# tgm-team/tgm

Hardware: AMD Instinct MI355X
Metric: sampled-edges/sec (TGAT 2-hop k=20 recency sampler, tgbl-wiki synthetic) (higher is better)
Workload: dtype int32/int64 indices + f32 feature rows (copied, no arithmetic)

## Files before the change

include/tgm_amd.h:

```cpp
#ifndef TGM_AMD_H
#define TGM_AMD_H

#include <stddef.h>
#include <stdint.h>

#ifdef __cplusplus
extern "C" {
#endif

#define TGMX_ABI_VERSION 7

#define TGMX_OK 0
#define TGMX_E_INVALID (-1)
#define TGMX_E_LAUNCH (-2)
#define TGMX_E_UNSUPPORTED (-3)

#define TGMX_ST_SEED_RANGE 1
#define TGMX_ST_SEED_TIME 2
#define TGMX_ST_EDGE_RANGE 4
#define TGMX_ST_SCRATCH 8
#define TGMX_ST_TS_BOUND 16

typedef void* tgmx_stream_t;
typedef void* tgmx_event_t;
// ... 80 lines not shown
  int64_t ts_bound;
  int32_t neg_group, neg_low, neg_high;
  uint64_t neg_seed, neg_call;
  int32_t* neg_out;
  int64_t* neg_time_out;
  int32_t guard_seed_errors;
  int32_t sorted_ts;
  int32_t* out_valid[TGMX_MAX_HOPS];
  int32_t* out_valid_prev[TGMX_MAX_HOPS];
  int64_t neg_index0;
  int64_t* csr_cursor;
  int32_t csr_x_by_pos;
  int32_t* out_eid[TGMX_MAX_HOPS];
  struct tgmx_defer* defer;
  int32_t defer_ok;
} tgmx_recency_step_t;

int tgmx_recency_step(const tgmx_recency_step_t* step, tgmx_stream_t stream);
#define TGMX_PLAN_FUSED01 1
#define TGMX_RIDE_NONE 0
#define TGMX_RIDE_SORT 1
#define TGMX_RIDE_MERGE 2
#define TGMX_RIDE_SORT_MERGE 3
#define TGMX_RIDE_PLACE_ONLY 4
#define TGMX_RIDE_ALL 5
#define TGMX_RIDE_SORT_MERGE_PLACE 6
#define TGMX_RIDE_MERGE_PLACE 7
#define TGMX_AFTER_NONE 0
#define TGMX_AFTER_COMMIT 1
#define TGMX_AFTER_PRESORTED 2
#define TGMX_AFTER_MERGE_PRESORTED 3
#define TGMX_AFTER_BLOCK 4
#define TGMX_AFTER_LARGE 5
int tgmx_recency_step_plan(const tgmx_recency_step_t* step);
// ... 28 lines not shown
} tgmx_pipeline_t;

typedef struct tgmx_pipeline_out {
  int32_t* neg;
  int64_t* neg_time;
  int32_t* seed_nid0;
  int64_t* seed_ts0;
  int32_t* out_nid[TGMX_MAX_HOPS];
  int64_t* out_ts[TGMX_MAX_HOPS];
  float* out_x[TGMX_MAX_HOPS];
  int32_t timed_hop;
  tgmx_event_t ev_start, ev_stop;
  int32_t* out_valid[TGMX_MAX_HOPS];
  int32_t* out_valid_prev[TGMX_MAX_HOPS];
  int32_t* out_eid[TGMX_MAX_HOPS];
} tgmx_pipeline_out_t;

typedef struct tgmx_pipeline_post {
  int32_t dedup;
  int32_t dedup_neg, dedup_nbr;
  int32_t num_nodes;
  void* dedup_ws;
  int32_t* uniq_out;
  int32_t edge_hop;
  int64_t edge_cap;
  int64_t* row_off;
  int64_t* edge_index;
  int64_t* edge_t;
  float* edge_x;
  int64_t* dev_sizes;
// ... 1032 lines not shown
```

tgm_amd/_native.py:

```python
from __future__ import annotations

import ctypes
import os
from ctypes import c_char_p, c_int32, c_int64, c_size_t, c_void_p
from typing import Optional

import torch

from .exceptions import NativeLibraryError

_HERE = os.path.dirname(os.path.abspath(__file__))
LIB_PATH = os.path.join(_HERE, 'csrc', 'libtgm_amd.so')

_P = c_void_p
SIGNATURES = {
    'tgmx_version': (c_int32, []),
    'tgmx_abi_sizeof': (c_size_t, [c_int32]),
    'tgmx_last_error': (c_char_p, []),
    'tgmx_event_create': (c_int32, [ctypes.POINTER(c_void_p)]),
    'tgmx_event_destroy': (c_int32, [_P]),
    'tgmx_event_elapsed_ms': (c_int32, [_P, _P, ctypes.POINTER(ctypes.c_float)]),
    'tgmx_recency_lookup_csr': (
        c_int32,
        [_P, _P, _P, c_int32, _P, _P, c_int64, c_int32, c_int32, c_int64, c_int64, c_int32, c_int32, _P, _P, _P, _P, _P, _P, _P],
# ... 129 lines not shown
        ('n_groups', c_int32),
        ('grp_nid', c_void_p * MAX_SEED_GROUPS), ('grp_ts', c_void_p * MAX_SEED_GROUPS), ('grp_n', c_int64 * MAX_SEED_GROUPS),
        ('seed_nid0', c_void_p), ('seed_ts0', c_void_p), ('S0', c_int64),
        ('n_hops', c_int32), ('k', c_int32 * MAX_HOPS),
        ('out_nid', c_void_p * MAX_HOPS), ('out_ts', c_void_p * MAX_HOPS), ('out_x', c_void_p * MAX_HOPS),
        ('src', c_void_p), ('dst', c_void_p), ('ts', c_void_p), ('edge_x', c_void_p),
        ('n', c_int64), ('eid0', c_int64), ('directed', c_int32), ('key_wrap32', c_int32),
        ('scratch', c_void_p), ('status', c_void_p),
        ('timed_hop', c_int32), ('ev_start', c_void_p), ('ev_stop', c_void_p),
        ('ts_bound', c_int64),
        ('neg_group', c_int32), ('neg_low', c_int32), ('neg_high', c_int32),
        ('neg_seed', ctypes.c_uint64), ('neg_call', ctypes.c_uint64), ('neg_out', c_void_p), ('neg_time_out', c_void_p),
        ('guard_seed_errors', c_int32), ('sorted_ts', c_int32),
        ('out_valid', c_void_p * MAX_HOPS), ('out_valid_prev', c_void_p * MAX_HOPS),
        ('neg_index0', c_int64), ('csr_cursor', c_void_p), ('csr_x_by_pos', c_int32), ('out_eid', c_void_p * MAX_HOPS),
        ('defer', c_void_p), ('defer_ok', c_int32),
    ]


class PipelinePost(ctypes.Structure):

    _fields_ = [
        ('dedup', c_int32), ('dedup_neg', c_int32), ('dedup_nbr', c_int32), ('num_nodes', c_int32), ('dedup_ws', c_void_p), ('uniq_out', c_void_p),
        ('edge_hop', c_int32), ('edge_cap', c_int64), ('row_off', c_void_p), ('edge_index', c_void_p), ('edge_t', c_void_p), ('edge_x', c_void_p),
        ('dev_sizes', c_void_p), ('host_sizes', c_void_p), ('sizes_ready', c_void_p),
    ]


class TgnMemoryFwd(ctypes.Structure):

    _fields_ = [
# ... 164 lines not shown
    _fields_ = [
        ('src', c_void_p), ('dst', c_void_p), ('ts', c_void_p), ('edge_x', c_void_p), ('num_edges', c_int64),
        ('rank', c_int32), ('world', c_int32), ('n_roles', c_int32), ('seed_role', c_int32 * MAX_SEED_GROUPS),
        ('neg_low', c_int32), ('neg_high', c_int32), ('neg_seed', ctypes.c_uint64),
        ('update', c_int32), ('reserved0', c_int32), ('step', RecencyStep),
    ]


class PipelineOut(ctypes.Structure):

    _fields_ = [
        ('neg', c_void_p), ('neg_time', c_void_p), ('seed_nid0', c_void_p), ('seed_ts0', c_void_p),
        ('out_nid', c_void_p * MAX_HOPS), ('out_ts', c_void_p * MAX_HOPS), ('out_x', c_void_p * MAX_HOPS),
        ('timed_hop', c_int32), ('ev_start', c_void_p), ('ev_stop', c_void_p),
        ('out_valid', c_void_p * MAX_HOPS), ('out_valid_prev', c_void_p * MAX_HOPS), ('out_eid', c_void_p * MAX_HOPS),
    ]


ACCOUNTING_PARTIALS = 1024
SIGNATURES['tgmx_lookup_accounting'] = (c_int32, [_P, c_int64, _P, _P, c_int64, _P, _P])
SIGNATURES['tgmx_uniform_lookup_csr'] = (c_int32, [_P, _P, _P, c_int32, _P, c_int64, c_int32, c_int64, c_int32, c_int32, ctypes.c_uint64, ctypes.c_uint64,
                                                   _P, _P, _P, _P, _P])
SIGNATURES['tgmx_ring_update_scratch_bytes'] = (c_size_t, [c_int64, c_int32])
SIGNATURES['tgmx_defer_create'] = (c_void_p, [c_int32, c_int32])
SIGNATURES['tgmx_defer_destroy'] = (None, [_P])
SIGNATURES['tgmx_defer_pending'] = (c_int32, [_P])
SIGNATURES['tgmx_defer_count'] = (c_int64, [_P])
SIGNATURES['tgmx_defer_flush'] = (c_int32, [_P, _P])
SIGNATURES['tgmx_set_fused_rows'] = (c_int32, [c_int32])
SIGNATURES['tgmx_set_fused_order'] = (c_int32, [c_int32])
SIGNATURES['tgmx_fused_row_order'] = (c_int32, [c_int64, c_int32, c_int32, _P, c_int32, _P])
SIGNATURES['tgmx_tgn_gru_gate_backward'] = (c_int32, [_P, _P, _P, _P, c_int32, c_int64, _P, _P, _P])
SIGNATURES['tgmx_tgn_aggregate_backward'] = (c_int32, [c_int64, _P, _P, _P, _P, _P, _P, c_int32, c_int32, _P, _P, c_int32, c_int32, _P, _P, _P])
SIGNATURES['tgmx_tconv_edge_attr_backward'] = (c_int32, [_P, _P, _P, _P, _P, _P, c_int32, c_int32, c_int64, _P, _P])
# ... 633 lines not shown
```

tgm_amd/csrc/pipeline.hip:

```cpp
#include <algorithm>

#include "common.h"

using namespace tgmx;

__global__ __launch_bounds__(64) void sizes_to_host_kernel(const int64_t* __restrict__ dev, int64_t* __restrict__ host) {
  if (threadIdx.x < 3) __hip_atomic_store(&host[threadIdx.x], dev[threadIdx.x], __ATOMIC_RELAXED, __HIP_MEMORY_SCOPE_SYSTEM);
}

static int pipeline_post(const tgmx_pipeline_t* p, const tgmx_recency_step_t& s, int64_t edge_lo, int64_t n_edges, long long share,
                         const tgmx_pipeline_out_t* out, const tgmx_pipeline_post_t* post, tgmx_stream_t stream) {
  TGMX_REQUIRE(post->dev_sizes && post->host_sizes && post->sizes_ready, "pipeline_step: post block needs dev_sizes / host_sizes / sizes_ready");
  long long rows[TGMX_MAX_HOPS + 1];
  rows[0] = share * p->n_roles;
  for (int h = 0; h < s.n_hops; ++h) rows[h + 1] = rows[h] * s.k[h];
  bool scan_rides = false;
  if (post->dedup) {
    TGMX_REQUIRE(post->dedup_ws && post->uniq_out, "pipeline_step: null dedup buffer");
    const int32_t* parts[16];
    int64_t sizes[16];
    int np = 0;
    parts[np] = p->src + edge_lo; sizes[np++] = n_edges;
    parts[np] = p->dst + edge_lo; sizes[np++] = n_edges;
    if (post->dedup_neg && s.neg_out) { parts[np] = s.neg_out; sizes[np++] = share; }
// ... 63 lines not shown
        s.neg_index0 = lo;
        s.neg_out = out->neg; s.neg_time_out = out->neg_time;
        break;
      default: TGMX_REQUIRE(false, "pipeline_step: seed role %d", p->seed_role[g]);
    }
  }
  s.seed_nid0 = out->seed_nid0;
  s.seed_ts0 = out->seed_ts0;
  for (int h = 0; h < s.n_hops && h < TGMX_MAX_HOPS; ++h) {
    s.out_nid[h] = out->out_nid[h];
    s.out_ts[h] = out->out_ts[h];
    s.out_x[h] = out->out_x[h];
    s.out_valid[h] = out->out_valid[h];
    s.out_valid_prev[h] = out->out_valid_prev[h];
    s.out_eid[h] = out->out_eid[h];
  }
  s.timed_hop = out->timed_hop;
  s.ev_start = out->ev_start;
  s.ev_stop = out->ev_stop;
  if (s.indptr) {
    s.ev_hi = edge_lo;
    s.n = 0;
  } else if (p->update && n_edges > 0) {
    s.src = p->src + edge_lo;
    s.dst = p->dst + edge_lo;
    s.ts = p->ts + edge_lo;
    s.edge_x = (p->edge_x && s.D > 0) ? p->edge_x + edge_lo * (long long)s.D : nullptr;
    s.n = n_edges;
    s.eid0 = edge_lo;
    s.defer_ok = 1;
// ... 58 lines not shown
```

tgm_amd/csrc/recency.hip:

```cpp
#include <algorithm>
#include <atomic>
#include <cstdlib>
#include <cstring>
#include <string>
#include <vector>

#include <hip/hip_ext.h>
#include <rocprim/block/block_radix_sort.hpp>
#include <rocprim/block/block_scan.hpp>
#include <rocprim/device/device_radix_sort.hpp>
#include <rocprim/device/device_scan.hpp>
#include <rocprim/iterator/counting_iterator.hpp>
#include <rocprim/iterator/transform_iterator.hpp>

#include "common.h"

namespace tgmx {

struct __align__(16) Rec {
  int nbr;
  int eid;
  long long ts;
};
static_assert(sizeof(Rec) == sizeof(tgmx_adj_t), "record layout");
// ... 108 lines not shown
  unsigned commit_blocks;
  const unsigned long long* phdr;
  const Rec* prec;
  const int32_t* pslot;
  const float* pstore;
  unsigned pstamp;
  int peid0;
  int k1;
  int32_t* out_nid1;
  int64_t* out_ts1;
  float* out_x1;
  int32_t* out_valid;
  int32_t* out_valid1;
  int32_t* out_valid_prev;
  int32_t* out_valid_prev1;
  int fused_rows;
  FusedOrder ord;
  long long* ts;
};

template <int VEC>
struct VecOf;
template <>
struct VecOf<4> { using type = float4; };
template <>
struct VecOf<2> { using type = float2; };
template <>
struct VecOf<1> { using type = float; };

template <typename T>
// ... 1123 lines not shown
      has[u] = e >= 0;
      const bool st = e >= lim;
      ptr[u] = (st ? P : X) + (has[u] ? (long long)(st ? e - lim : e) * a.row_vecs + col : 0);
    }
    V v[U];
#pragma unroll
    for (int u = 0; u < U; ++u) v[u] = *ptr[u];
#pragma unroll
    for (int u = 0; u < U; ++u) {
      const int f = f0 + u * kWave;
      if (f < total) O[f] = has[u] ? v[u] : zero_vec<V>();
    }
  }
}

template <bool RING, int VEC, bool SMALL, bool PRE = false>
__device__ __forceinline__ void lookup_seed(const LookupArgs& a, long long s, int n, long long q, int k, int lane, int* lds_eid,
                                            int32_t* out_nid, int64_t* out_ts, float* out_x, int32_t* out_valid, int32_t* out_valid_prev,
                                            int32_t* out_eid = nullptr, int v_old_pre = 0) {
  const bool live = n >= 0 && n < a.N;
  int v_new = 0;
  if (SMALL) {
    const SmallPick o = small_pick<RING>(a, n, q, k, live, lane);
    if (lane < k) {
      out_nid[s * k + lane] = o.nbr;
      out_ts[s * k + lane] = o.ts;
      if (out_eid) out_eid[s * k + lane] = o.eid;
      lds_eid[lane] = o.src;
    }
    const unsigned long long m = __ballot(lane < k && o.has);
    v_new = m ? k - __builtin_ctzll(m) : 0;
  } else {
    const int B = a.B;
    const Window w = find_window<RING>(a, n, live, lane);
    int cnt = 0;
    for (int top = w.wlen; top > 0 && cnt == 0; top -= kWave) {
      const int lo = top > kWave ? top - kWave : 0;
      const int i = lo + lane;
      bool ok = false;
      if (i < top) {
        const Rec r = a.recs[slot_of<RING>(w, B, i)];
        ok = r.nbr >= 0 && r.ts < q;
      }
      const unsigned long long m = __ballot(ok);
      if (m) cnt = lo + 64 - __clzll((long long)m);
    }
    for (int c = lane; c < k; c += kWave) {
      const int i = cnt - k + c;
      Rec r;
      r.nbr = -1; r.eid = 0; r.ts = 0;
      if (i >= 0) r = a.recs[slot_of<RING>(w, B, i)];
      const bool has = r.nbr >= 0;
      out_nid[s * k + c] = has ? r.nbr : -1;
      out_ts[s * k + c] = has ? r.ts : 0;
      if (out_eid) out_eid[s * k + c] = has ? r.eid : -1;
      lds_eid[c] = has ? ((RING || a.x_by_pos) ? (int)slot_of<RING>(w, B, i) : r.eid) : -1;
      if (has && k - c > v_new) v_new = k - c;
    }
    for (int o = 32; o > 0; o >>= 1) {
      const int other = __shfl_xor(v_new, o);
      v_new = other > v_new ? other : v_new;
    }
  }
  if (a.D == 0 || out_x == nullptr) return;
  int first_slot = 0;
  if (out_valid) {
    const int v_old = PRE ? v_old_pre : out_valid[s];
    first_slot = k - (v_old > v_new ? v_old : v_new);
    if (lane == 0) {
      out_valid[s] = v_new;
      if (out_valid_prev) out_valid_prev[s] = v_old;
    }
  }
  __builtin_amdgcn_wave_barrier();
  gather_rows<VEC>(a, s, k, lane, lds_eid, out_x, first_slot);
  __builtin_amdgcn_wave_barrier();
}

template <bool RING, int VEC, bool SMALL, bool RIDE>
__global__ __launch_bounds__(256) void recency_lookup_kernel(const LookupArgs a, const UpdateArgs u) {
  extern __shared__ __attribute__((aligned(16))) int lds_eid_all[];
  unsigned bid = blockIdx.x, nblk = gridDim.x;
  if constexpr (RING && RIDE) {
    if (bid < a.side_blocks) {
      update_side_work(u, a.side_stage, (int)bid);
      return;
    }
    bid -= a.side_blocks;
    nblk -= a.side_blocks;
  }
  const int lane = lane_id();
  const int wave_in_block = threadIdx.x >> 6;
  int* lds_eid = lds_eid_all + wave_in_block * a.k;
  const long long waves_total = (long long)nblk * (blockDim.x >> 6);
  for (long long s = (long long)bid * (blockDim.x >> 6) + wave_in_block; s < a.S; s += waves_total) {
    int n;
    long long q;
    fetch_seed(a, s, lane, true, n, q);
    check_seed(a, n, q, a.allow_pad, lane);
    lookup_seed<RING, VEC, SMALL>(a, s, n, q, a.k, lane, lds_eid, a.out_nid, a.out_ts, a.out_x, a.out_valid, a.out_valid_prev, a.out_eid);
  }
}

constexpr int kFusedTsWords = 8;
constexpr int kFusedRowsDefault = 0;
enum FusedTsRole : long long { kTsRider = 1, kTsCommit = 2, kTsHop0 = 3, kTsHop1 = 4 };
__device__ __forceinline__ long long ts_after(int v) {
  asm volatile("" ::"v"(v));
  return (long long)wall_clock64();
}

template <bool RING>
__device__ __forceinline__ SmallPick fused_row_pick(const LookupArgs& a, const PickLoads& L, int n, long long q, bool live, int lane) {
  if constexpr (RING) return pick_finish(a, L, n, q, a.k1, live, lane);
  else return small_pick<false>(a, n, q, a.k1, live, lane);
// ... 33 lines not shown
  const int k0 = a.k, k1 = a.k1;
  int* lds_eid = lds_eid_all + wave_in_block * (k0 > k1 ? k0 : k1);
  const long long waves_total = (long long)nblk * (blockDim.x >> 6);
  const long long S0 = a.S;
  const int G = ROWS ? a.fused_rows : 0;
  const int runs = G > 0 ? (k0 + G - 1) / G : k0;
  long long role = 0, t_seed = 0, t_index = 0, t_gather = 0, ts_row = -1;
  for (long long w = (long long)bid * (blockDim.x >> 6) + wave_in_block; w < S0 + S0 * runs; w += waves_total) {
    int n;
    long long q;
    if (w < S0) {
      role = kTsHop0;
      if constexpr (ROWS) {
        fetch_seed(a, w, lane, true, n, q);
        check_seed(a, n, q, 0, lane);
        lookup_seed<RING, VEC, true>(a, w, n, q, k0, lane, lds_eid, a.out_nid, a.out_ts, a.out_x, a.out_valid, a.out_valid_prev, a.out_eid);
      } else {
        const int v_old = (a.D > 0 && a.out_x && a.out_valid) ? a.out_valid[w] : 0;
        fetch_seed(a, w, lane, true, n, q);
        check_seed(a, n, q, 0, lane);
        lookup_seed<RING, VEC, true, true>(a, w, n, q, k0, lane, lds_eid, a.out_nid, a.out_ts, a.out_x, a.out_valid, a.out_valid_prev, a.out_eid, v_old);
      }
    } else if (!ROWS) {
      role = kTsHop1;
      long long s0;
      int j;
      fused_row_of(a.ord, w - S0, k0, S0, s0, j);
      const long long idx = s0 * k0 + j;
      const int v_old = (a.D > 0 && a.out_x1 && a.out_valid1) ? a.out_valid1[idx] : 0;
      if (TS) ts_row = idx;
      int n0;
      long long q0;
      fetch_seed(a, s0, lane, false, n0, q0);
      const SmallPick o = small_pick<RING>(a, n0, q0, k0, n0 >= 0 && n0 < a.N, lane);
      n = __shfl(o.nbr, j);
      q = __shfl(o.ts, j);
      lookup_seed<RING, VEC, true, true>(a, idx, n, q, k1, lane, lds_eid, a.out_nid1, a.out_ts1, a.out_x1, a.out_valid1, a.out_valid_prev1, a.out_eid1, v_old);
    } else {
      const long long run = w - S0;
      const long long s0 = run / runs;
      const int j0 = (int)(run - s0 * runs) * G;
      const int rows = k0 - j0 < G ? k0 - j0 : G;
      const long long base = s0 * k0 + j0;
      const bool feats = a.D > 0 && a.out_x1 != nullptr;
      const int v_old_run = (feats && a.out_valid1 && lane < rows) ? a.out_valid1[base + lane] : 0;
      int n0;
      long long q0;
      fetch_seed(a, s0, lane, false, n0, q0);
      const SmallPick o0 = small_pick<RING>(a, n0, q0, k0, n0 >= 0 && n0 < a.N, lane);
      n = __shfl(o0.nbr, j0);
      q = __shfl(o0.ts, j0);
      bool live = n >= 0 && n < a.N;
// ... 2 lines not shown
        t_seed = ts_after(n);
      }
      PickLoads L = RING ? pick_issue(a, n, live, lane) : PickLoads{};
      for (int r = 0; r < rows; ++r) {
        const long long s = base + r;
        const long long t0 = TS ? (long long)wall_clock64() : 0;
        const SmallPick o = fused_row_pick<RING>(a, L, n, q, live, lane);
        if (lane < k1) {
          a.out_nid1[s * k1 + lane] = o.nbr;
          a.out_ts1[s * k1 + lane] = o.ts;
          if (a.out_eid1) a.out_eid1[s * k1 + lane] = o.eid;
          lds_eid[lane] = o.src;
        }
        const unsigned long long m = __ballot(lane < k1 && o.has);
        const int v_new = m ? k1 - __builtin_ctzll(m) : 0;
        if (TS) {
          const long long t1 = ts_after(v_new);
          t_index += t1 - t0;
        }
        if (r + 1 < rows) {
          n = __shfl(o0.nbr, j0 + r + 1);
          q = __shfl(o0.ts, j0 + r + 1);
          live = n >= 0 && n < a.N;
          if (RING) L = pick_issue(a, n, live, lane);
        }
        if (!feats) continue;
        int first_slot = 0;
        if (a.out_valid1) {
          const int v_old = __shfl(v_old_run, r);
          first_slot = k1 - (v_old > v_new ? v_old : v_new);
          if (lane == 0) {
            a.out_valid1[s] = v_new;
            if (a.out_valid_prev1) a.out_valid_prev1[s] = v_old;
          }
        }
        const long long t2 = TS ? (long long)wall_clock64() : 0;
        __builtin_amdgcn_wave_barrier();
        gather_rows<VEC>(a, s, k1, lane, lds_eid, a.out_x1, first_slot);
        __builtin_amdgcn_wave_barrier();
        if (TS) t_gather += (long long)wall_clock64() - t2;
      }
    }
  }
  if (TS && lane == 0) {
    ts_rec[0] = t_start;
    ts_rec[1] = (long long)wall_clock64();
    ts_rec[2] = role;
    ts_rec[3] = t_seed;
// ... 673 lines not shown
  a.row_vecs = a.D > 0 ? a.D / vec : 1;
  a.dv = make_fastdiv((uint32_t)a.row_vecs);
  a.dv_seed = make_fastdiv((uint32_t)(kmax * a.row_vecs));
  if ((unsigned long long)kmax * a.row_vecs * (unsigned long long)a.row_vecs >= (1ull << 32)) {
    set_error("recency_lookup: k*D^2 too large for the slot divider (k=%d, D=%d)", kmax, a.D);
    return TGMX_E_UNSUPPORTED;
  }
  return vec;
}

static int packed_group_lanes(const LookupArgs& a, int k, bool ring) {
  const int gl = (a.B <= 16 && k <= 16) ? 16 : ((a.B <= 32 && k <= 32) ? 32 : 64);
  return (ring && gl < 64 && (long long)k * a.row_vecs <= 8 * gl) ? gl : 64;
}

template <bool RING>
static int launch_lookup(LookupArgs a, hipStream_t stream, hipEvent_t ev_start, hipEvent_t ev_stop,
                         const UpdateArgs* side = nullptr, int side_stage = 0, unsigned side_blocks = 0) {
  if (a.S == 0) return TGMX_OK;
  const UpdateArgs u = side ? *side : UpdateArgs{};
  a.side_blocks = (RING && side) ? side_blocks : 0;
  a.side_stage = side_stage;
  const bool small = a.B <= kWave && a.k <= kWave;
  const int vec = prepare_lookup(a, a.out_x, a.k);
  if (vec < 0) return vec;
  const int waves_per_block = 4;
  long long blocks = (a.S + waves_per_block - 1) / waves_per_block;
  if (blocks > (1 << 20)) blocks = 1 << 20;
  const dim3 grid((unsigned)blocks + a.side_blocks), block(waves_per_block * kWave);
  const size_t lds = (size_t)waves_per_block * a.k * sizeof(int);
  const bool ride = RING && a.side_blocks > 0;
#define TGMX_LAUNCH(VEC_, SMALL_)                                                                                              \
  do {                                                                                                                         \
    if (ride) TGMX_LAUNCH_TIMED((recency_lookup_kernel<RING, VEC_, SMALL_, true>), grid, block, lds, stream, ev_start, ev_stop, a, u); \
    else TGMX_LAUNCH_TIMED((recency_lookup_kernel<RING, VEC_, SMALL_, false>), grid, block, lds, stream, ev_start, ev_stop, a, u);     \
  } while (0)
  const int gl_any = a.out_eid ? 64 : packed_group_lanes(a, a.k, true);
  static const bool packed_hop0 = !(getenv("TGMX_PACKED_HOP0") && atoi(getenv("TGMX_PACKED_HOP0")) == 0);
  const int gl = (a.grp.groups == 0 || packed_hop0) ? gl_any : 64;
  static const bool tile_on = !(getenv("TGMX_TILE") && atoi(getenv("TGMX_TILE")) == 0);
  const bool tile_ok = gl_any < 64 && tile_on && a.B <= 32 && a.k <= 32 && (((uintptr_t)a.out_nid | (uintptr_t)a.out_ts) & 15) == 0 &&
                       a.S <= (1ll << 25) && a.S >= 2ll * kWave * device_cu_count() &&
                       (!RING || (long long)a.N * a.B * (a.D > 0 ? a.D : 1) * 4 < (1ll << 32) - 64);
  if (tile_ok) {
    const int wpb = ride ? 4 : 1;
    const long long tiles = (a.S + kWave - 1) / kWave;
    long long tblocks = (tiles + wpb - 1) / wpb;
    if (a.leave_room && !ride) {
      const long long room = (long long)device_cu_count() * 12;
      if (tblocks > room) tblocks = room;
    }
    const dim3 tgrid((unsigned)tblocks + a.side_blocks), tblock(wpb * kWave);
// ... 989 lines not shown
  if (n_hops == 1) return {{kSideSort}, {chunks}, 0, kAfterMergePresorted};
  if (chunks == 1) return {{kSideSortMerge, kSidePlaceOnly}, {1, 1}, 0, kAfterCommit};
  if (m <= kRidePlaceMaxM) return {{kSideSort, kSideMergePlace}, {chunks, chunks}, 0, kAfterCommit};
  return {{kSideSort, kSideMerge}, {chunks, chunks}, 0, kAfterPresorted};
}

static long long hop0_seed_count(const tgmx_recency_step_t* s) {
  if (s->n_groups <= 0) return s->S0;
  long long S = 0;
  for (int g = 0; g < s->n_groups && g < TGMX_MAX_SEED_GROUPS; ++g) S += s->grp_n[g];
  return S;
}

static long long ring_entries(const tgmx_recency_step_t* s) { return s->n <= 0 ? 0 : (s->directed ? s->n : 2 * s->n); }

extern "C" int tgmx_recency_step_plan(const tgmx_recency_step_t* s) {
  if (!s) return 0;
  const long long S = hop0_seed_count(s);
  const bool fused = plan_fuse01(s, S);
  const RiderPlan p = plan_riders(ring_entries(s), s->n_hops, S, fused, s->indptr == nullptr);
  return (fused ? TGMX_PLAN_FUSED01 : 0) | p.stage[0] << 4 | p.stage[1] << 8 | (int)p.blocks[0] << 12 | (int)p.blocks[1] << 17 |
         (p.pcap / 512) << 22 | p.after << 24;
}

static LookupArgs step_lookup_args(const tgmx_recency_step_t* s) {
  LookupArgs a{};
  a.indptr = s->indptr; a.recs = reinterpret_cast<const Rec*>(s->ring); a.write_pos = s->write_pos; a.edge_x = s->ring_x;
  a.status = s->status; a.D = s->D; a.B = s->B; a.N = s->num_nodes;
  a.ev_lo = s->ev_lo; a.ev_hi = s->ev_hi;
  a.x_by_pos = s->indptr && s->csr_x_by_pos;
  return a;
}

extern "C" int tgmx_recency_step(const tgmx_recency_step_t* s, tgmx_stream_t stream) {
  TGMX_REQUIRE(s, "recency_step: null argument block");
  TGMX_REQUIRE(s->n_groups >= 0 && s->n_groups <= TGMX_MAX_SEED_GROUPS && s->n_hops >= 0 && s->n_hops <= TGMX_MAX_HOPS,
// ... 78 lines not shown

  const int32_t* cur_n = s->seed_nid0;
  const int64_t* cur_t = s->seed_ts0;
  int h = 0;
  if (fused) {
    const int k0 = s->k[0], k1 = s->k[1];
    TGMX_REQUIRE(s->B >= k0 && s->B >= k1, "recency_step: k=[%d, %d] but B=%d", k0, k1, s->B);
    TGMX_REQUIRE(cur_n && cur_t && s->out_nid[0] && s->out_ts[0] && s->out_nid[1] && s->out_ts[1] &&
                     (s->D == 0 || (s->ring_x && (s->out_x[0] || s->out_eid[0]) && (s->out_x[1] || s->out_eid[1]))), "recency_step: null pointer at hop 0 / 1");
    LookupArgs a = step_lookup_args(s);
    a.grp = grp;
    a.seeds = cur_n; a.qtimes = cur_t; a.out_nid = s->out_nid[0]; a.out_ts = s->out_ts[0]; a.out_x = s->out_x[0];
    a.k1 = k1; a.out_nid1 = s->out_nid[1]; a.out_ts1 = s->out_ts[1]; a.out_x1 = s->out_x[1];
    a.out_valid = s->out_valid[0]; a.out_valid1 = s->out_valid[1];
    a.out_valid_prev = s->out_valid_prev[0]; a.out_valid_prev1 = s->out_valid_prev[1];
    a.out_eid = s->out_eid[0]; a.out_eid1 = s->out_eid[1];
    a.S = S; a.k = k0; a.allow_pad = 0;
    const bool timed = s->timed_hop == 0 || s->timed_hop == 1;
    hipEvent_t e0 = timed ? (hipEvent_t)s->ev_start : nullptr, e1 = timed ? (hipEvent_t)s->ev_stop : nullptr;
    const bool commit = defer && dfr->pending;
    if (commit) {
      a.phdr = u.phdr; a.pstamp = u.pstamp;
      a.prec = dfr->rec[(stamp & 1) ^ 1]; a.pslot = dfr->slot[(stamp & 1) ^ 1];
      a.pstore = s->D > 0 ? dfr->pend.edge_x : nullptr; a.peid0 = (int)dfr->pend.eid0;
    }
    const int rc = csr ? launch_fused01<false>(a, st, e0, e1, nullptr, 0, 0, 0)
                       : launch_fused01<true>(a, st, e0, e1, plan.blocks[0] > 0 ? &u : nullptr, plan.stage[0], plan.blocks[0], plan.pcap,
                                              commit ? &dfr->pend : nullptr);
    if (rc) return rc;
    if (const int rs = enqueue_side()) return rs;
    cur_n = s->out_nid[1];
    cur_t = s->out_ts[1];
    S *= (long long)k0 * k1;
    h = 2;
  }
  for (; h < s->n_hops && S > 0; ++h) {
    const int k = s->k[h];
    TGMX_REQUIRE(k > 0 && s->B >= k, "recency_step: hop %d has k=%d, B=%d", h, k, s->B);
    TGMX_REQUIRE(cur_n && cur_t && s->out_nid[h] && s->out_ts[h] && (s->D == 0 || (s->ring_x && (s->out_x[h] || s->out_eid[h]))),
                 "recency_step: null pointer at hop %d", h);
    LookupArgs a = step_lookup_args(s);
    if (h == 0) a.grp = grp;
    a.seeds = cur_n; a.qtimes = cur_t; a.out_nid = s->out_nid[h]; a.out_ts = s->out_ts[h]; a.out_x = s->out_x[h];
    a.out_valid = s->out_valid[h]; a.out_valid_prev = s->out_valid_prev[h];
    a.out_eid = s->out_eid[h];
    a.S = S; a.k = k; a.allow_pad = h > 0;
    a.cursor = csr ? reinterpret_cast<long long*>(s->csr_cursor) : nullptr;
    a.leave_room = side != nullptr;
    const bool timed = h == s->timed_hop;
    hipEvent_t e0 = timed ? (hipEvent_t)s->ev_start : nullptr, e1 = timed ? (hipEvent_t)s->ev_stop : nullptr;
    const bool ride = h < 2 && plan.blocks[h] > 0;
    const int rc = csr ? launch_lookup<false>(a, st, e0, e1)
                       : launch_lookup<true>(a, st, e0, e1, ride ? &u : nullptr, ride ? plan.stage[h] : 0, ride ? plan.blocks[h] : 0u);
    if (rc) return rc;
    if (const int rs = enqueue_side()) return rs;
    cur_n = s->out_nid[h];
    cur_t = s->out_ts[h];
    S *= k;
  }
// ... 36 lines not shown
```

tgm_amd/hooks/recency.py:

```python
from __future__ import annotations

import ctypes
import logging
import os
import warnings
import weakref
from typing import Dict, List, Optional, Sequence

import torch
from torch import Tensor

from .. import _native
from ..core import DGBatch, DGraph
from ..index import TemporalCSR, build_csr
from .base import SeedableHook, StatefulHook
from .registry import hook

logger = logging.getLogger('tgm_amd.hooks.recency')

_ST_SEED_RANGE, _ST_SEED_TIME, _ST_EDGE_RANGE, _ST_SCRATCH, _ST_TS_BOUND = 1, 2, 4, 8, 16


class _NullCtx:
    def __enter__(self):
        return None

    def __exit__(self, *exc):
        return False


_NULL = _NullCtx()


def _on_device(device: torch.device):
    idx = device.index
    cur = _native._cuda_get_device
    if idx is None or idx == (cur() if cur is not None else torch.cuda.current_device()):
        return _NULL
    return torch.cuda.device(device)


@hook
class RecencyNeighborHook(StatefulHook, SeedableHook):

    _cls_requires = {'edge_src', 'edge_dst', 'edge_time'}
    _cls_produces = {'seed_nids', 'seed_times', 'nbr_nids', 'nbr_edge_time', 'nbr_edge_x', 'seed_node_nbr_mask'}
# ... 481 lines not shown
                    ex = None
                src, dst, tt = batch.edge_src, batch.edge_dst, batch.edge_time
                if not (src.is_contiguous() and dst.is_contiguous() and tt.is_contiguous()):
                    src, dst, tt = src.contiguous(), dst.contiguous(), tt.contiguous()
                keep = (src, dst, tt, ex)
                st.src, st.dst, st.ts, st.edge_x = src.data_ptr(), dst.data_ptr(), tt.data_ptr(), _native.ptr(ex)
                st.eid0 = -1 if batch._edge_lo is None else int(batch._edge_lo)
                slice_ = self._is_store_slice(batch, tt, device)
                st.ts_bound, st.sorted_ts = self._store_promise if slice_ else (0, 0)
                if slice_ and self._defer is not None and batch._edge_lo is not None:
                    sx = self._bound_store.on(device).edge_x if D else None
                    st.defer_ok = 1 if (ex is None or (sx is not None and ex.data_ptr() == sx.data_ptr() + 4 * D * int(batch._edge_lo))) else 0

            st.n, st.n_hops = n_edges, L
            st.guard_seed_errors = 1 if self._validate == 'sync' else 0
            rc = lib.tgmx_recency_step(st, stream)
            if rc:
                _native.check(rc, 'tgmx_recency_step')
            if self._validate == 'sync':
                self.check()
            del keep
            if timer is not None:
                hops = [0, 1] if self.profile_hop in (0, 1) and self.fuses_first_hops() else [self.profile_hop]
                counts = torch.empty(len(hops), dtype=torch.int64, device=device)
                for i, h in enumerate(hops):
                    torch.sum((out_n[h] != -1).view(-1), dim=0, dtype=torch.int64, out=counts[i])
                self.profile_log.append((timer, [(out_seed_n[h].shape[0], self._num_nbrs[h]) for h in hops], counts, None))
        if by_id:
            from ..core.lazy import EdgeFeaturesById

            out_x = EdgeFeaturesById(out_eid, self._feature_table(dg, device))
        return self._publish(batch, out_seed_n, out_seed_t, out_n, out_t, out_x, seed_mask)

    def _feature_table(self, dg: DGraph, device: torch.device) -> Tensor:
        return dg._storage.on(device).edge_x

    def _get_seed_tensors(self, batch: DGBatch, device: torch.device, concat: bool = True):
        seeds: List[Tensor] = []
        times: List[Tensor] = []
        mask: Dict[str, Tensor] = {}
        offset = 0
# ... 55 lines not shown
```

tgm_amd/pipeline.py:

```python
from __future__ import annotations

import ctypes
import os
import sys
import weakref
from typing import Dict, List, Optional, Sequence

import torch

from . import _native
from .core import DGBatch, DGraph
from .dist import EdgeShardHook, shard_bounds
from .hooks.dedup import DeduplicationHook
from .hooks.edge_list import SampledEdgeListHook
from .hooks.negatives import RandomNegativeEdgeSamplerHook
from .hooks.recency import RecencyNeighborHook

_ROLE_KEYS = {
    False: {'edge_src': (_native.SEED_SRC, 'edge_time'), 'edge_dst': (_native.SEED_DST, 'edge_time'), 'neg': (_native.SEED_NEG, 'neg_time')},
    True: {'shard_src': (_native.SEED_SRC, 'shard_time'), 'shard_dst': (_native.SEED_DST, 'shard_time'), 'neg': (_native.SEED_NEG, 'neg_time')},
}


_STATUS_READ_EVERY = 512
_TAGGED = frozenset(('seed_nids', 'seed_times', 'nbr_nids', 'nbr_edge_time', 'nbr_edge_x'))
_MAX_AUTO_SETS = 4
_storage_uses = torch._C._storage_Use_Count


def _snapshot(tensors: list) -> list:
    return [(sys.getrefcount(t), t._use_count()) for t in tensors]


class _Slot:

    __slots__ = ('out', 'attrs', 'nbr_nids', 'post', 'post_bufs', 'valid', 'watch', 'base')


class _OutputSet:

    __slots__ = ('buf', 'cap', 'off', 'views', 'storage', 'uses', 'version', 'pin', 'event', 'arange_n', 'lib', 'stream')

    def __del__(self) -> None:
        ev, lib = getattr(self, 'event', None), getattr(self, 'lib', None)
        if ev and lib is not None:
            try:
                lib.tgmx_event_destroy(ev)
            except Exception:
                pass


# ... 109 lines not shown
            pos = (pos + nbytes + 255) & ~255

        take('neg', 4 * share)
        take('neg_time', 8 * share)
        take('seeds', 4 * S0)
        take('seed_t', 8 * S0)
        take('arange', 8 * S0)
        S = S0
        total_ids = 0
        for hop, k in enumerate(nbr._num_nbrs):
            take(f'nid{hop}', 4 * S * k)
            take(f'nts{hop}', 8 * S * k)
            take(f'nx{hop}', 0 if nbr._by_id else 4 * S * k * D)
            take(f'eid{hop}', 4 * S * k if nbr._by_id else 0)
            take(f'nv{hop}', 4 * S)
            take(f'nvp{hop}', 4 * S)
            total_ids += S * k
            S *= k
        if self._dedup is not None:
            N = int(self._dg._storage.num_nodes_global)
            extra = set(self._dedup.seed_keys or [])
            total = 2 * cap + (share if 'neg' in extra else 0) + (total_ids if 'nbr_nids' in extra else 0)
            take('uniq', 4 * max(min(total, N), 1))
            take('dev_sizes', 24)
            if self._edges is not None:
                h = self._edges.hop
                Sh = S0
                for k in nbr._num_nbrs[:h]:
                    Sh *= k
                ecap = max(Sh * nbr._num_nbrs[h], 1)
                take('ei', 16 * ecap)
# ... 64 lines not shown
            out.neg, out.neg_time = neg_t.data_ptr(), negt_t.data_ptr()
            attrs['neg'], attrs['neg_time'] = neg_t, negt_t
        seeds, seed_t = view('seeds', torch.int32, S0), view('seed_t', torch.int64, S0)
        out.seed_nid0, out.seed_ts0 = seeds.data_ptr(), seed_t.data_ptr()
        seed_n, seed_ts, nbr_n, nbr_t, nbr_x, valid = [], [], [], [], [], []
        cur_n, cur_t, S = seeds, seed_t, S0
        for hop, k in enumerate(nbr._num_nbrs):
            nid, nts = view(f'nid{hop}', torch.int32, S, k), view(f'nts{hop}', torch.int64, S, k)
            by_id = nbr._by_id and D > 0
            if by_id:
                nx = view(f'eid{hop}', torch.int32, S, k)
                out.out_eid[hop] = nx.data_ptr()
            else:
                nx = view(f'nx{hop}', torch.float32, S, k, D)
            if self._delta and not by_id:
                o, op = off[f'nv{hop}'], off[f'nvp{hop}']
                nv = (buf[o:o + 4 * S].view(torch.int32), buf[op:op + 4 * S].view(torch.int32))
                out.out_valid[hop], out.out_valid_prev[hop] = nv[0].data_ptr(), nv[1].data_ptr()
                valid.append(nv)
            out.out_nid[hop], out.out_ts[hop], out.out_x[hop] = nid.data_ptr(), nts.data_ptr(), (0 if by_id else nx.data_ptr())
            seed_n.append(cur_n)
            seed_ts.append(cur_t)
            nbr_n.append(nid)
            nbr_t.append(nts)
            nbr_x.append(nx)
            if hop + 1 < len(nbr._num_nbrs):
                cur_n, cur_t = nid.view(-1), nts.view(-1)
                watch += [cur_n, cur_t]
            S *= k
        whole = view('arange', torch.int64, S0)
        mask = {}
        for g, key in enumerate(nbr._seed_nodes_keys):
            mask[key] = whole.narrow(0, g * share, share)
            watch.append(mask[key])
        attrs.update(seed_nids=seed_n, seed_times=seed_ts, nbr_nids=nbr_n, nbr_edge_time=nbr_t, nbr_edge_x=nbr_x, seed_node_nbr_mask=mask)
        sl.out, sl.attrs, sl.nbr_nids, sl.valid = out, attrs, nbr_n, valid
        sl.post = sl.post_bufs = None
        if self._dedup is not None:
            sl.post, sl.post_bufs = self._make_post(os_, n, share, nbr_n)
        sl.watch, sl.base = watch, None
        os_.views[n] = sl
        return sl

    def _baseline(self, os_: _OutputSet, sl: _Slot) -> None:
        sl.base = _snapshot(sl.watch)
        os_.uses = _storage_uses(os_.storage._cdata)

    def _make_post(self, os_: _OutputSet, n: int, share: int, nbr_n):
        nbr, buf, off = self._nbr, os_.buf, os_.off
        N = int(self._dg._storage.num_nodes_global)
        extra = set(self._dedup.seed_keys or [])
        total = 2 * n + (share if 'neg' in extra else 0) + (sum(t.numel() for t in nbr_n) if 'nbr_nids' in extra else 0)
# ... 117 lines not shown
                nbr._epoch_lo = lo
            st = pipe.step
            st.indptr, st.ring, st.ring_x, st.ev_lo = nbr._step.indptr, nbr._step.ring, nbr._step.ring_x, nbr._epoch_lo
            st.csr_cursor, st.csr_x_by_pos = nbr._step.csr_cursor, nbr._step.csr_x_by_pos
        nbr._note_batch_time(self._dg, batch)
        call = 0
        neg = self._neg
        if neg is not None:
            call = neg._calls = neg._calls + 1
        out = slot.out
        nbr._calls += 1
        timer = None
        if nbr.profile_hop is not None and nbr._calls % nbr.profile_every == 0 and nbr.profile_pool:
            timer = nbr.profile_pool.pop()
            out.timed_hop, out.ev_start, out.ev_stop = nbr.profile_hop, timer.start, timer.stop
        asy = self._async
        if asy is not None and timer is None:
            tk = ctypes.c_uint64()
            rc = self._lib.tgmx_worker_pipeline_step(asy[0], pipe, lo, n, call, out, slot.post, _native.stream_ptr(self._device.index), asy[1], asy[2],
                                                     ctypes.byref(tk))
            if rc:
                _native.check(rc, 'tgmx_worker_pipeline_step')
            batch.__dict__['_ticket'] = self._last_ticket = tk.value
        else:
            stream = _native.stream_ptr(self._device.index)
            self._order_behind_worker()
            rc = self._lib.tgmx_pipeline_step(pipe, lo, n, call, out, slot.post, stream)
            if rc:
                _native.check(rc, 'tgmx_pipeline_step')
        if timer is not None:
            out.timed_hop = -1
            self._log_timed(timer, slot)
        if nbr._validate == 'sync':
            self._since_check += 1
            if not self._static_ok[0] or self._since_check >= _STATUS_READ_EVERY:
                self._since_check = 0
                if asy is not None and self._last_ticket:
                    _native.check(self._lib.tgmx_worker_wait(asy[0], self._last_ticket), 'tgmx_worker_wait')
                nbr.check()
        d = batch.__dict__
        if shard is not None:
            arr = self._arr
            d['shard_src'] = arr.src.narrow(0, lo + s_lo, s_hi - s_lo)
            d['shard_dst'] = arr.dst.narrow(0, lo + s_lo, s_hi - s_lo)
            d['shard_time'] = arr.ts.narrow(0, lo + s_lo, s_hi - s_lo)
            d['shard_lo'] = s_lo
        from .core.lazy import EdgeFeaturesById, SampledHops, SamplerCallTag
# ... 43 lines not shown
        N = nbr._num_nodes
        if self._neg is not None and not (0 <= self._neg.low and self._neg.high <= N):
            return (False,)
        with torch.cuda.device(self._device):
            oob = lambda t: (t < 0) | (t >= N)
            bad_src, bad_dst = oob(arr.src), oob(arr.dst)
            seed = torch.zeros_like(bad_src)
            if _native.SEED_SRC in self._roles:
                seed |= bad_src
            if _native.SEED_DST in self._roles:
                seed |= bad_dst
            idx = lambda m: m.nonzero().view(-1).cpu().numpy()
            edge = (bad_src | bad_dst) if nbr._mode == 'ring' else torch.zeros_like(bad_src)
            return (True, idx(seed), idx(arr.ts < 0), idx(edge))

    def _log_timed(self, timer, slot: _Slot) -> None:
        nbr = self._nbr
        st = self._pipe.step
        st.n_groups, st.S0 = 0, slot.attrs['seed_nids'][0].shape[0]
        for h in range(len(nbr._num_nbrs)):
            st.out_x[h] = slot.out.out_x[h]
        fused = bool(self._lib.tgmx_recency_step_plan(st) & 1)
        hops = [0, 1] if nbr.profile_hop in (0, 1) and fused else [nbr.profile_hop]
        parts = torch.empty((len(hops), _native.ACCOUNTING_PARTIALS, 3), dtype=torch.int64, device=self._device)
        stream = _native.stream_ptr(self._device.index)
        for i, h in enumerate(hops):
            ids = slot.nbr_nids[h]
            sp = slot.valid[h] if slot.valid else None
            _native.check(self._lib.tgmx_lookup_accounting(ids.data_ptr(), ids.numel(), sp[1].data_ptr() if sp is not None else None,
                                                           sp[0].data_ptr() if sp is not None else None, ids.shape[0], parts[i].data_ptr(), stream),
                          'tgmx_lookup_accounting')
        nbr.profile_log.append((timer, [(slot.attrs['seed_nids'][h].shape[0], nbr._num_nbrs[h]) for h in hops], _Counts(parts, 0),
                                _Counts(parts, 1) if slot.valid else None))


class _Counts:

    def __init__(self, parts: torch.Tensor, col: int) -> None:
        self._parts, self._col = parts, col

    def sum(self) -> torch.Tensor:
        return self._parts[:, :, self._col].sum()
```

Baseline: 9.809 billion.

## Compute profiling accounting inline in lookup kernel and drop per-step valid_prev buffer

For timed (profiled) calls, the lookup kernel now writes a packed per-seed accounting word (valid count, max old/new window, new window) directly, replacing the separate accounting kernel or torch reduction run afterward. The always-allocated out_valid_prev buffer is removed from the pipeline and only provided on profiled calls, which cuts output memory and writes on ordinary steps. This adds extra shuffles and branches in the lookup inner loop when accounting is enabled, and makes the plan function build lookup args to decide inline eligibility.

```diff
diff --git a/include/tgm_amd.h b/include/tgm_amd.h
--- a/include/tgm_amd.h
+++ b/include/tgm_amd.h
@@ -118,10 +118,12 @@
   int32_t* out_eid[TGMX_MAX_HOPS];
   struct tgmx_defer* defer;
   int32_t defer_ok;
+  int64_t* out_acct[TGMX_MAX_HOPS];
 } tgmx_recency_step_t;
 
 int tgmx_recency_step(const tgmx_recency_step_t* step, tgmx_stream_t stream);
 #define TGMX_PLAN_FUSED01 1
+#define TGMX_ACCT_INLINE 2
 #define TGMX_RIDE_NONE 0
 #define TGMX_RIDE_SORT 1
 #define TGMX_RIDE_MERGE 2
@@ -180,6 +182,7 @@
   int32_t* out_valid[TGMX_MAX_HOPS];
   int32_t* out_valid_prev[TGMX_MAX_HOPS];
   int32_t* out_eid[TGMX_MAX_HOPS];
+  int64_t* out_acct[TGMX_MAX_HOPS];
 } tgmx_pipeline_out_t;
 
 typedef struct tgmx_pipeline_post {
diff --git a/tgm_amd/_native.py b/tgm_amd/_native.py
--- a/tgm_amd/_native.py
+++ b/tgm_amd/_native.py
@@ -167,7 +167,7 @@
         ('guard_seed_errors', c_int32), ('sorted_ts', c_int32),
         ('out_valid', c_void_p * MAX_HOPS), ('out_valid_prev', c_void_p * MAX_HOPS),
         ('neg_index0', c_int64), ('csr_cursor', c_void_p), ('csr_x_by_pos', c_int32), ('out_eid', c_void_p * MAX_HOPS),
-        ('defer', c_void_p), ('defer_ok', c_int32),
+        ('defer', c_void_p), ('defer_ok', c_int32), ('out_acct', c_void_p * MAX_HOPS),
     ]
 
 
@@ -362,10 +362,12 @@
         ('out_nid', c_void_p * MAX_HOPS), ('out_ts', c_void_p * MAX_HOPS), ('out_x', c_void_p * MAX_HOPS),
         ('timed_hop', c_int32), ('ev_start', c_void_p), ('ev_stop', c_void_p),
         ('out_valid', c_void_p * MAX_HOPS), ('out_valid_prev', c_void_p * MAX_HOPS), ('out_eid', c_void_p * MAX_HOPS),
+        ('out_acct', c_void_p * MAX_HOPS),
     ]
 
 
 ACCOUNTING_PARTIALS = 1024
+PLAN_FUSED01, ACCT_INLINE = 1, 2
 SIGNATURES['tgmx_lookup_accounting'] = (c_int32, [_P, c_int64, _P, _P, c_int64, _P, _P])
 SIGNATURES['tgmx_uniform_lookup_csr'] = (c_int32, [_P, _P, _P, c_int32, _P, c_int64, c_int32, c_int64, c_int32, c_int32, ctypes.c_uint64, ctypes.c_uint64,
                                                    _P, _P, _P, _P, _P])
diff --git a/tgm_amd/csrc/pipeline.hip b/tgm_amd/csrc/pipeline.hip
--- a/tgm_amd/csrc/pipeline.hip
+++ b/tgm_amd/csrc/pipeline.hip
@@ -101,6 +101,7 @@
     s.out_valid[h] = out->out_valid[h];
     s.out_valid_prev[h] = out->out_valid_prev[h];
     s.out_eid[h] = out->out_eid[h];
+    s.out_acct[h] = out->out_acct[h];
   }
   s.timed_hop = out->timed_hop;
   s.ev_start = out->ev_start;
diff --git a/tgm_amd/csrc/recency.hip b/tgm_amd/csrc/recency.hip
--- a/tgm_amd/csrc/recency.hip
+++ b/tgm_amd/csrc/recency.hip
@@ -146,6 +146,8 @@
   int32_t* out_valid1;
   int32_t* out_valid_prev;
   int32_t* out_valid_prev1;
+  int64_t* out_acct;
+  int64_t* out_acct1;
   int fused_rows;
   FusedOrder ord;
   long long* ts;
@@ -1299,12 +1301,17 @@
   }
 }
 
+__device__ __forceinline__ long long acct_word(int count, int v_old, int v_new) {
+  return (long long)count | (long long)(v_old > v_new ? v_old : v_new) << 21 | (long long)v_new << 42;
+}
+
 template <bool RING, int VEC, bool SMALL, bool PRE = false>
 __device__ __forceinline__ void lookup_seed(const LookupArgs& a, long long s, int n, long long q, int k, int lane, int* lds_eid,
                                             int32_t* out_nid, int64_t* out_ts, float* out_x, int32_t* out_valid, int32_t* out_valid_prev,
-                                            int32_t* out_eid = nullptr, int v_old_pre = 0) {
+                                            int32_t* out_eid = nullptr, int v_old_pre = 0, int64_t* out_acct = nullptr) {
   const bool live = n >= 0 && n < a.N;
   int v_new = 0;
+  int count = 0;
   if (SMALL) {
     const SmallPick o = small_pick<RING>(a, n, q, k, live, lane);
     if (lane < k) {
@@ -1315,6 +1322,7 @@
     }
     const unsigned long long m = __ballot(lane < k && o.has);
     v_new = m ? k - __builtin_ctzll(m) : 0;
+    count = __popcll(m);
   } else {
     const int B = a.B;
     const Window w = find_window<RING>(a, n, live, lane);
@@ -1341,13 +1349,17 @@
       if (out_eid) out_eid[s * k + c] = has ? r.eid : -1;
       lds_eid[c] = has ? ((RING || a.x_by_pos) ? (int)slot_of<RING>(w, B, i) : r.eid) : -1;
       if (has && k - c > v_new) v_new = k - c;
+      count += has;
     }
     for (int o = 32; o > 0; o >>= 1) {
       const int other = __shfl_xor(v_new, o);
       v_new = other > v_new ? other : v_new;
-    }
-  }
-  if (a.D == 0 || out_x == nullptr) return;
+      if (out_acct) count += __shfl_xor(count, o);
+    }
+  }
+  const bool feats = a.D > 0 && out_x != nullptr;
+  if (out_acct && lane == 0 && !(feats && out_valid)) out_acct[s] = acct_word(count, 0, 0);
+  if (!feats) return;
   int first_slot = 0;
   if (out_valid) {
     const int v_old = PRE ? v_old_pre : out_valid[s];
@@ -1355,6 +1367,7 @@
     if (lane == 0) {
       out_valid[s] = v_new;
       if (out_valid_prev) out_valid_prev[s] = v_old;
+      if (out_acct) out_acct[s] = acct_word(count, v_old, v_new);
     }
   }
   __builtin_amdgcn_wave_barrier();
@@ -1383,7 +1396,7 @@
     long long q;
     fetch_seed(a, s, lane, true, n, q);
     check_seed(a, n, q, a.allow_pad, lane);
-    lookup_seed<RING, VEC, SMALL>(a, s, n, q, a.k, lane, lds_eid, a.out_nid, a.out_ts, a.out_x, a.out_valid, a.out_valid_prev, a.out_eid);
+    lookup_seed<RING, VEC, SMALL>(a, s, n, q, a.k, lane, lds_eid, a.out_nid, a.out_ts, a.out_x, a.out_valid, a.out_valid_prev, a.out_eid, 0, a.out_acct);
   }
 }
 
@@ -1447,12 +1460,12 @@
       if constexpr (ROWS) {
         fetch_seed(a, w, lane, true, n, q);
         check_seed(a, n, q, 0, lane);
-        lookup_seed<RING, VEC, true>(a, w, n, q, k0, lane, lds_eid, a.out_nid, a.out_ts, a.out_x, a.out_valid, a.out_valid_prev, a.out_eid);
+        lookup_seed<RING, VEC, true>(a, w, n, q, k0, lane, lds_eid, a.out_nid, a.out_ts, a.out_x, a.out_valid, a.out_valid_prev, a.out_eid, 0, a.out_acct);
       } else {
         const int v_old = (a.D > 0 && a.out_x && a.out_valid) ? a.out_valid[w] : 0;
         fetch_seed(a, w, lane, true, n, q);
         check_seed(a, n, q, 0, lane);
-        lookup_seed<RING, VEC, true, true>(a, w, n, q, k0, lane, lds_eid, a.out_nid, a.out_ts, a.out_x, a.out_valid, a.out_valid_prev, a.out_eid, v_old);
+        lookup_seed<RING, VEC, true, true>(a, w, n, q, k0, lane, lds_eid, a.out_nid, a.out_ts, a.out_x, a.out_valid, a.out_valid_prev, a.out_eid, v_old, a.out_acct);
       }
     } else if (!ROWS) {
       role = kTsHop1;
@@ -1468,7 +1481,7 @@
       const SmallPick o = small_pick<RING>(a, n0, q0, k0, n0 >= 0 && n0 < a.N, lane);
       n = __shfl(o.nbr, j);
       q = __shfl(o.ts, j);
-      lookup_seed<RING, VEC, true, true>(a, idx, n, q, k1, lane, lds_eid, a.out_nid1, a.out_ts1, a.out_x1, a.out_valid1, a.out_valid_prev1, a.out_eid1, v_old);
+      lookup_seed<RING, VEC, true, true>(a, idx, n, q, k1, lane, lds_eid, a.out_nid1, a.out_ts1, a.out_x1, a.out_valid1, a.out_valid_prev1, a.out_eid1, v_old, a.out_acct1);
     } else {
       const long long run = w - S0;
       const long long s0 = run / runs;
@@ -1501,6 +1514,7 @@
         }
         const unsigned long long m = __ballot(lane < k1 && o.has);
         const int v_new = m ? k1 - __builtin_ctzll(m) : 0;
+        if (a.out_acct1 && lane == 0 && !(feats && a.out_valid1)) a.out_acct1[s] = acct_word(__popcll(m), 0, 0);
         if (TS) {
           const long long t1 = ts_after(v_new);
           t_index += t1 - t0;
@@ -1519,6 +1533,7 @@
           if (lane == 0) {
             a.out_valid1[s] = v_new;
             if (a.out_valid_prev1) a.out_valid_prev1[s] = v_old;
+            if (a.out_acct1) a.out_acct1[s] = acct_word(__popcll(m), v_old, v_new);
           }
         }
         const long long t2 = TS ? (long long)wall_clock64() : 0;
@@ -2222,6 +2237,8 @@
   return (ring && gl < 64 && (long long)k * a.row_vecs <= 8 * gl) ? gl : 64;
 }
 
+static int narrow_group_lanes(const LookupArgs& a) { return a.out_eid ? 64 : packed_group_lanes(a, a.k, true); }
+
 template <bool RING>
 static int launch_lookup(LookupArgs a, hipStream_t stream, hipEvent_t ev_start, hipEvent_t ev_stop,
                          const UpdateArgs* side = nullptr, int side_stage = 0, unsigned side_blocks = 0) {
@@ -2243,7 +2260,7 @@
     if (ride) TGMX_LAUNCH_TIMED((recency_lookup_kernel<RING, VEC_, SMALL_, true>), grid, block, lds, stream, ev_start, ev_stop, a, u); \
     else TGMX_LAUNCH_TIMED((recency_lookup_kernel<RING, VEC_, SMALL_, false>), grid, block, lds, stream, ev_start, ev_stop, a, u);     \
   } while (0)
-  const int gl_any = a.out_eid ? 64 : packed_group_lanes(a, a.k, true);
+  const int gl_any = narrow_group_lanes(a);
   static const bool packed_hop0 = !(getenv("TGMX_PACKED_HOP0") && atoi(getenv("TGMX_PACKED_HOP0")) == 0);
   const int gl = (a.grp.groups == 0 || packed_hop0) ? gl_any : 64;
   static const bool tile_on = !(getenv("TGMX_TILE") && atoi(getenv("TGMX_TILE")) == 0);
@@ -3263,12 +3280,21 @@
 
 static long long ring_entries(const tgmx_recency_step_t* s) { return s->n <= 0 ? 0 : (s->directed ? s->n : 2 * s->n); }
 
+static bool plan_acct_inline(const tgmx_recency_step_t* s, int h, bool fused) {
+  if (h < 0 || h >= s->n_hops || h >= TGMX_MAX_HOPS || s->k[h] <= 0) return false;
+  if (fused && h < 2) return true;
+  LookupArgs a{};
+  a.B = s->B; a.D = s->D; a.k = s->k[h]; a.edge_x = s->ring_x; a.out_x = s->out_x[h]; a.out_eid = s->out_eid[h];
+  if (prepare_lookup(a, a.out_x, a.k) < 0) return false;
+  return narrow_group_lanes(a) == 64;
+}
+
 extern "C" int tgmx_recency_step_plan(const tgmx_recency_step_t* s) {
   if (!s) return 0;
   const long long S = hop0_seed_count(s);
   const bool fused = plan_fuse01(s, S);
   const RiderPlan p = plan_riders(ring_entries(s), s->n_hops, S, fused, s->indptr == nullptr);
-  return (fused ? TGMX_PLAN_FUSED01 : 0) | p.stage[0] << 4 | p.stage[1] << 8 | (int)p.blocks[0] << 12 | (int)p.blocks[1] << 17 |
+  return (fused ? TGMX_PLAN_FUSED01 : 0) | (plan_acct_inline(s, s->timed_hop, fused) ? TGMX_ACCT_INLINE : 0) | p.stage[0] << 4 | p.stage[1] << 8 | (int)p.blocks[0] << 12 | (int)p.blocks[1] << 17 |
          (p.pcap / 512) << 22 | p.after << 24;
 }
 
@@ -3377,6 +3403,7 @@
     a.k1 = k1; a.out_nid1 = s->out_nid[1]; a.out_ts1 = s->out_ts[1]; a.out_x1 = s->out_x[1];
     a.out_valid = s->out_valid[0]; a.out_valid1 = s->out_valid[1];
     a.out_valid_prev = s->out_valid_prev[0]; a.out_valid_prev1 = s->out_valid_prev[1];
+    a.out_acct = s->out_acct[0]; a.out_acct1 = s->out_acct[1];
     a.out_eid = s->out_eid[0]; a.out_eid1 = s->out_eid[1];
     a.S = S; a.k = k0; a.allow_pad = 0;
     const bool timed = s->timed_hop == 0 || s->timed_hop == 1;
@@ -3405,7 +3432,7 @@
     LookupArgs a = step_lookup_args(s);
     if (h == 0) a.grp = grp;
     a.seeds = cur_n; a.qtimes = cur_t; a.out_nid = s->out_nid[h]; a.out_ts = s->out_ts[h]; a.out_x = s->out_x[h];
-    a.out_valid = s->out_valid[h]; a.out_valid_prev = s->out_valid_prev[h];
+    a.out_valid = s->out_valid[h]; a.out_valid_prev = s->out_valid_prev[h]; a.out_acct = s->out_acct[h];
     a.out_eid = s->out_eid[h];
     a.S = S; a.k = k; a.allow_pad = h > 0;
     a.cursor = csr ? reinterpret_cast<long long*>(s->csr_cursor) : nullptr;
diff --git a/tgm_amd/hooks/recency.py b/tgm_amd/hooks/recency.py
--- a/tgm_amd/hooks/recency.py
+++ b/tgm_amd/hooks/recency.py
@@ -30,6 +30,15 @@
 
 
 _NULL = _NullCtx()
+
+
+class AcctField:
+
+    def __init__(self, words: Tensor, col: int) -> None:
+        self._words, self._shift = words, 21 * col
+
+    def sum(self) -> Tensor:
+        return ((self._words >> self._shift) & 0x1FFFFF).sum()
 
 
 def _on_device(device: torch.device):
@@ -541,17 +550,32 @@
 
             st.n, st.n_hops = n_edges, L
             st.guard_seed_errors = 1 if self._validate == 'sync' else 0
+            words = None
+            if timer is not None:
+                plan = lib.tgmx_recency_step_plan(st)
+                hops = [0, 1] if self.profile_hop in (0, 1) and plan & _native.PLAN_FUSED01 else [self.profile_hop]
+                if plan & _native.ACCT_INLINE:
+                    words = torch.empty(sum(out_n[h].shape[0] for h in hops), dtype=torch.int64, device=device)
+                    at = words.data_ptr()
+                    for h in hops:
+                        st.out_acct[h] = at
+                        at += 8 * out_n[h].shape[0]
             rc = lib.tgmx_recency_step(st, stream)
+            if words is not None:
+                for h in hops:
+                    st.out_acct[h] = None
             if rc:
                 _native.check(rc, 'tgmx_recency_step')
             if self._validate == 'sync':
                 self.check()
             del keep
             if timer is not None:
-                hops = [0, 1] if self.profile_hop in (0, 1) and self.fuses_first_hops() else [self.profile_hop]
-                counts = torch.empty(len(hops), dtype=torch.int64, device=device)
-                for i, h in enumerate(hops):
-                    torch.sum((out_n[h] != -1).view(-1), dim=0, dtype=torch.int64, out=counts[i])
+                if words is not None:
+                    counts = AcctField(words, 0)
+                else:
+                    counts = torch.empty(len(hops), dtype=torch.int64, device=device)
+                    for i, h in enumerate(hops):
+                        torch.sum((out_n[h] != -1).view(-1), dim=0, dtype=torch.int64, out=counts[i])
                 self.profile_log.append((timer, [(out_seed_n[h].shape[0], self._num_nbrs[h]) for h in hops], counts, None))
         if by_id:
             from ..core.lazy import EdgeFeaturesById
diff --git a/tgm_amd/pipeline.py b/tgm_amd/pipeline.py
--- a/tgm_amd/pipeline.py
+++ b/tgm_amd/pipeline.py
@@ -14,7 +14,7 @@
 from .hooks.dedup import DeduplicationHook
 from .hooks.edge_list import SampledEdgeListHook
 from .hooks.negatives import RandomNegativeEdgeSamplerHook
-from .hooks.recency import RecencyNeighborHook
+from .hooks.recency import AcctField, RecencyNeighborHook
 
 _ROLE_KEYS = {
     False: {'edge_src': (_native.SEED_SRC, 'edge_time'), 'edge_dst': (_native.SEED_DST, 'edge_time'), 'neg': (_native.SEED_NEG, 'neg_time')},
@@ -34,7 +34,7 @@
 
 class _Slot:
 
-    __slots__ = ('out', 'attrs', 'nbr_nids', 'post', 'post_bufs', 'valid', 'watch', 'base')
+    __slots__ = ('out', 'attrs', 'nbr_nids', 'post', 'post_bufs', 'valid', 'prev', 'watch', 'base')
 
 
 class _OutputSet:
@@ -174,7 +174,6 @@
             take(f'nx{hop}', 0 if nbr._by_id else 4 * S * k * D)
             take(f'eid{hop}', 4 * S * k if nbr._by_id else 0)
             take(f'nv{hop}', 4 * S)
-            take(f'nvp{hop}', 4 * S)
             total_ids += S * k
             S *= k
         if self._dedup is not None:
@@ -269,9 +268,9 @@
             else:
                 nx = view(f'nx{hop}', torch.float32, S, k, D)
             if self._delta and not by_id:
-                o, op = off[f'nv{hop}'], off[f'nvp{hop}']
-                nv = (buf[o:o + 4 * S].view(torch.int32), buf[op:op + 4 * S].view(torch.int32))
-                out.out_valid[hop], out.out_valid_prev[hop] = nv[0].data_ptr(), nv[1].data_ptr()
+                o = off[f'nv{hop}']
+                nv = buf[o:o + 4 * S].view(torch.int32)
+                out.out_valid[hop] = nv.data_ptr()
                 valid.append(nv)
             out.out_nid[hop], out.out_ts[hop], out.out_x[hop] = nid.data_ptr(), nts.data_ptr(), (0 if by_id else nx.data_ptr())
             seed_n.append(cur_n)
@@ -290,7 +289,7 @@
             watch.append(mask[key])
         attrs.update(seed_nids=seed_n, seed_times=seed_ts, nbr_nids=nbr_n, nbr_edge_time=nbr_t, nbr_edge_x=nbr_x, seed_node_nbr_mask=mask)
         sl.out, sl.attrs, sl.nbr_nids, sl.valid = out, attrs, nbr_n, valid
-        sl.post = sl.post_bufs = None
+        sl.post = sl.post_bufs = sl.prev = None
         if self._dedup is not None:
             sl.post, sl.post_bufs = self._make_post(os_, n, share, nbr_n)
         sl.watch, sl.base = watch, None
@@ -438,6 +437,7 @@
         if nbr.profile_hop is not None and nbr._calls % nbr.profile_every == 0 and nbr.profile_pool:
             timer = nbr.profile_pool.pop()
             out.timed_hop, out.ev_start, out.ev_stop = nbr.profile_hop, timer.start, timer.stop
+            acct = self._begin_timed(slot)
         asy = self._async
         if asy is not None and timer is None:
             tk = ctypes.c_uint64()
@@ -450,11 +450,14 @@
             stream = _native.stream_ptr(self._device.index)
             self._order_behind_worker()
             rc = self._lib.tgmx_pipeline_step(pipe, lo, n, call, out, slot.post, stream)
+            if timer is not None:
+                for h in acct[0]:
+                    out.out_acct[h] = out.out_valid_prev[h] = None
             if rc:
                 _native.check(rc, 'tgmx_pipeline_step')
         if timer is not None:
             out.timed_hop = -1
-            self._log_timed(timer, slot)
+            self._log_timed(timer, slot, acct)
         if nbr._validate == 'sync':
             self._since_check += 1
             if not self._static_ok[0] or self._since_check >= _STATUS_READ_EVERY:
@@ -528,24 +531,47 @@
             edge = (bad_src | bad_dst) if nbr._mode == 'ring' else torch.zeros_like(bad_src)
             return (True, idx(seed), idx(arr.ts < 0), idx(edge))
 
-    def _log_timed(self, timer, slot: _Slot) -> None:
-        nbr = self._nbr
+    def _begin_timed(self, slot: _Slot) -> tuple:
+        nbr, out = self._nbr, slot.out
         st = self._pipe.step
         st.n_groups, st.S0 = 0, slot.attrs['seed_nids'][0].shape[0]
         for h in range(len(nbr._num_nbrs)):
-            st.out_x[h] = slot.out.out_x[h]
-        fused = bool(self._lib.tgmx_recency_step_plan(st) & 1)
-        hops = [0, 1] if nbr.profile_hop in (0, 1) and fused else [nbr.profile_hop]
+            st.out_x[h], st.out_eid[h] = out.out_x[h], out.out_eid[h]
+        st.timed_hop = nbr.profile_hop
+        plan = self._lib.tgmx_recency_step_plan(st)
+        st.timed_hop = -1
+        hops = [0, 1] if nbr.profile_hop in (0, 1) and plan & _native.PLAN_FUSED01 else [nbr.profile_hop]
+        if plan & _native.ACCT_INLINE:
+            rows = [slot.nbr_nids[h].shape[0] for h in hops]
+            words = torch.empty(sum(rows), dtype=torch.int64, device=self._device)
+            at = words.data_ptr()
+            for h, r in zip(hops, rows):
+                out.out_acct[h] = at
+                at += 8 * r
+            return hops, words
+        if slot.valid:
+            if slot.prev is None:
+                slot.prev = [torch.zeros_like(v) for v in slot.valid]
+            for h in hops:
+                out.out_valid_prev[h] = slot.prev[h].data_ptr()
+        return hops, None
+
+    def _log_timed(self, timer, slot: _Slot, acct: tuple) -> None:
+        nbr = self._nbr
+        hops, words = acct
+        shapes = [(slot.attrs['seed_nids'][h].shape[0], nbr._num_nbrs[h]) for h in hops]
+        if words is not None:
+            nbr.profile_log.append((timer, shapes, AcctField(words, 0), AcctField(words, 1) if slot.valid else None))
+            return
         parts = torch.empty((len(hops), _native.ACCOUNTING_PARTIALS, 3), dtype=torch.int64, device=self._device)
         stream = _native.stream_ptr(self._device.index)
         for i, h in enumerate(hops):
             ids = slot.nbr_nids[h]
-            sp = slot.valid[h] if slot.valid else None
-            _native.check(self._lib.tgmx_lookup_accounting(ids.data_ptr(), ids.numel(), sp[1].data_ptr() if sp is not None else None,
-                                                           sp[0].data_ptr() if sp is not None else None, ids.shape[0], parts[i].data_ptr(), stream),
+            sp = (slot.prev[h], slot.valid[h]) if slot.valid else None
+            _native.check(self._lib.tgmx_lookup_accounting(ids.data_ptr(), ids.numel(), sp[0].data_ptr() if sp is not None else None,
+                                                           sp[1].data_ptr() if sp is not None else None, ids.shape[0], parts[i].data_ptr(), stream),
                           'tgmx_lookup_accounting')
-        nbr.profile_log.append((timer, [(slot.attrs['seed_nids'][h].shape[0], nbr._num_nbrs[h]) for h in hops], _Counts(parts, 0),
-                                _Counts(parts, 1) if slot.valid else None))
+        nbr.profile_log.append((timer, shapes, _Counts(parts, 0), _Counts(parts, 1) if slot.valid else None))
 
 
 class _Counts:
```

Measured after the change: 9.802 billion. Within noise of the previous version (-0.1%).
